# reglab/aquaculture

Hardware: AMD Instinct MI355X
Metric: 640px tiles/sec (whole node) YOLOv5m bf16 (higher is better)
Workload: dtype bf16

## Files before the change

aquaculture_amd/csrc/conv1x1_direct.hip:

```cpp
#include "conv_device.h"

using namespace aqdev;

namespace {

struct C1Params {
    const char* in;
    char* out;
    const char* w;
    const float* bias;
    const char* zero;
    int in_ld_b, out_ld_b;
    int npix, n_tiles, act;
    float out_inv_scale;
};

constexpr int kNW = 12;

template <int KS, int MBT, int MBW, int NBW> struct C1Geom {
    static constexpr int CIN = 32 * KS, COUT = 16 * MBT, CB = CIN / 8;
    static constexpr int MG = MBT / MBW;
    static constexpr int PG = kNW / MG;
    static constexpr int TP = PG * NBW * 16;
    static constexpr int SPP = CB + 2;
    static constexpr int PXB = SPP * 16;
    static constexpr int NQ = (TP * SPP + 63) / 64;
    static constexpr int XPB = NQ * 1024;
    static constexpr int LDS = 2 * XPB + COUT * 4;
    static constexpr int NST = NBW;
    static_assert(MBT % MBW == 0 && kNW % MG == 0 && LDS <= 160 * 1024, "shape");
};

__device__ __forceinline__ f32x4 c1_silu4(f32x4 v) {
    const f32x4 t = v * -1.44269504f;
    f32x4 d = {__builtin_amdgcn_exp2f(t[0]), __builtin_amdgcn_exp2f(t[1]), __builtin_amdgcn_exp2f(t[2]), __builtin_amdgcn_exp2f(t[3])};
    d = d + 1.0f;
    const f32x4 r = {__builtin_amdgcn_rcpf(d[0]), __builtin_amdgcn_rcpf(d[1]), __builtin_amdgcn_rcpf(d[2]), __builtin_amdgcn_rcpf(d[3])};
    return v * r;
}

template <int KS, int MBT, int MBW, int NBW, bool F8OUT = false>
__global__ __launch_bounds__(kNW * 64) void conv1x1_direct_kernel(const C1Params p) {
    using G = C1Geom<KS, MBT, MBW, NBW>;
    extern __shared__ __attribute__((aligned(16))) char smem[];
    float* s_b = (float*)(smem + 2 * G::XPB);

    const int tid = threadIdx.x, lane = tid & 63;
    const int wave = __builtin_amdgcn_readfirstlane(tid >> 6);
    static_assert(MBW == 2, "the paired-row layout below is written for two M blocks per wave");
    const int mb0 = (wave % G::MG) * MBW, pg = wave / G::MG;
    const int g = lane >> 4, l15 = lane & 15;
    const int cbase = mb0 * 16 + g * 8;

    bf16x8 wv[KS][MBW];
#pragma unroll
    for (int s = 0; s < KS; ++s)
#pragma unroll
        for (int m = 0; m < MBW; ++m) wv[s][m] = ((const bf16x8*)p.w)[((size_t)(mb0 + m) * KS + s) * 64 + lane];
    for (int i = tid; i < G::COUT; i += kNW * 64) s_b[i] = p.bias[i];

    auto issue_dma = [&](int tile, char* xb) {
        const long long n0 = (long long)tile * G::TP;
#pragma unroll 1
        for (int q = wave; q < G::NQ; q += kNW) {
            const int slot = q * 64 + lane;
            const int px = slot / G::SPP, part = slot - px * G::SPP;
            const bool valid = px < G::TP && part < G::CB && n0 + px < p.npix;
            const char* src = p.in + (n0 + px) * p.in_ld_b + part * 16;
            glds16(valid ? src : p.zero, xb + q * 1024);
        }
    };

    int tile = first_tile(gridDim.x, blockIdx.x);
    if (tile < p.n_tiles) issue_dma(tile, smem);
    int cur = 0;
    bool prev_full = false;
    for (; tile < p.n_tiles; tile += gridDim.x, cur ^= 1) {
        const long long n0 = (long long)tile * G::TP;
        const char* s_x = smem + cur * G::XPB;
        if (prev_full) wait_vmcnt<G::NST>(); else wait_vmcnt<0>();
        asm volatile("s_waitcnt lgkmcnt(0)" ::: "memory");
        __builtin_amdgcn_s_barrier();
        asm volatile("" ::: "memory");
        prev_full = n0 + G::TP <= p.npix;
        if (tile + (int)gridDim.x < p.n_tiles) issue_dma(tile + (int)gridDim.x, smem + (cur ^ 1) * G::XPB);

        f32x4 bv[MBW];
#pragma unroll
        for (int m = 0; m < MBW; ++m) bv[m] = *(const f32x4*)(s_b + cbase + m * 4);
        static_assert(G::NST == NBW * 1, "one 16-byte (8-byte with F8OUT) store per pixel block: the wait at the top of the tile loop counts these");
        AQ_STORE_LOOP_UNROLL
        for (int j = 0; j < NBW; ++j) {
            const int px = (pg * NBW + j) * 16 + l15;
            const char* base = s_x + px * G::PXB + g * 16;
            bf16x8 f[KS];
#pragma unroll
            for (int s = 0; s < KS; ++s) f[s] = *(const bf16x8*)(base + s * 64);
            f32x4 acc[MBW];
#pragma unroll
            for (int m = 0; m < MBW; ++m) acc[m] = f32x4{0.f, 0.f, 0.f, 0.f};
#pragma unroll
            for (int s = 0; s < KS; ++s)
#pragma unroll
                for (int m = 0; m < MBW; ++m) acc[m] = __builtin_amdgcn_mfma_f32_16x16x32_bf16(wv[s][m], f[s], acc[m], 0, 0, 0);
            f32x4 v0 = acc[0] + bv[0], v1 = acc[1] + bv[1];
            if (p.act) { v0 = c1_silu4(v0); v1 = c1_silu4(v1); }
            if constexpr (F8OUT) {
                f32x4 q0 = v0 * p.out_inv_scale, q1 = v1 * p.out_inv_scale;
#pragma unroll
                for (int e = 0; e < 4; ++e) {
                    q0[e] = __builtin_amdgcn_fmed3f(q0[e], -448.0f, 448.0f);
                    q1[e] = __builtin_amdgcn_fmed3f(q1[e], -448.0f, 448.0f);
                }
                int w0 = __builtin_amdgcn_cvt_pk_fp8_f32(q0[0], q0[1], 0, false);
                w0 = __builtin_amdgcn_cvt_pk_fp8_f32(q0[2], q0[3], w0, true);
                int w1 = __builtin_amdgcn_cvt_pk_fp8_f32(q1[0], q1[1], 0, false);
                w1 = __builtin_amdgcn_cvt_pk_fp8_f32(q1[2], q1[3], w1, true);
                if (n0 + px < p.npix) *(uint2*)(p.out + (n0 + px) * p.out_ld_b + cbase) = make_uint2((unsigned)w0, (unsigned)w1);
            } else if (n0 + px < p.npix)
                *(uint4*)(p.out + (n0 + px) * p.out_ld_b + cbase * 2) =
                    make_uint4(pack_bf16x2(v0[0], v0[1]), pack_bf16x2(v0[2], v0[3]), pack_bf16x2(v1[0], v1[1]), pack_bf16x2(v1[2], v1[3]));
        }
    }
}

template <int KS, int MBT, int MBW, int NBW, bool F8OUT = false>
int launch_c1(C1Params p, hipStream_t stream) {
    using G = C1Geom<KS, MBT, MBW, NBW>;
    auto fn = conv1x1_direct_kernel<KS, MBT, MBW, NBW, F8OUT>;
    int cus = 0;
    AQ_CHECK_HIP(aq_kernel_lds((const void*)fn, G::LDS));
    AQ_CHECK_HIP(aq_cus(&cus));
    p.n_tiles = (p.npix + G::TP - 1) / G::TP;
    long long grid = cus;
    if (grid > p.n_tiles) grid = p.n_tiles;
    hipLaunchKernelGGL(fn, dim3((unsigned)grid), dim3(kNW * 64), G::LDS, stream, p);
    AQ_CHECK_HIP(hipGetLastError());
    return AQ_OK;
}

}

extern "C" int aq_conv1x1_direct_supported(int cin, int cout) {
    return (cin == 96 && cout == 96) || (cin == 192 && cout == 192) || (cin == 384 && (cout == 192 || cout == 384));
}

extern "C" int aq_pack_conv1x1_direct(const float* w_host, int cin, int cout, void* packed_dev, size_t* bytes, void* stream) {
    AQ_REQUIRE(w_host && bytes && aq_conv1x1_direct_supported(cin, cout), "pack_conv1x1_direct: unsupported %d -> %d", cin, cout);
    const int ks = cin / 32, mbt = cout / 16;
    *bytes = (size_t)mbt * ks * 64 * 16;
    if (!packed_dev) return AQ_OK;
    bf16_t* host = (bf16_t*)calloc(1, *bytes);
    AQ_REQUIRE(host, "pack_conv1x1_direct: out of host memory");
    for (int mb = 0; mb < mbt; ++mb)
        for (int s = 0; s < ks; ++s)
            for (int lane = 0; lane < 64; ++lane) {
                const int r = lane & 15, g = lane >> 4;
                const int co = (mb >> 1) * 32 + 8 * (r >> 2) + 4 * (mb & 1) + (r & 3);
                bf16_t* dst = host + (((size_t)mb * ks + s) * 64 + lane) * 8;
                for (int e = 0; e < 8; ++e) dst[e] = aq_f2bf(w_host[(size_t)co * cin + 32 * s + 8 * g + e]);
            }
    hipError_t e = hipMemcpyAsync(packed_dev, host, *bytes, hipMemcpyHostToDevice, (hipStream_t)stream);
    if (e == hipSuccess) e = hipStreamSynchronize((hipStream_t)stream);
    free(host);
    AQ_CHECK_HIP(e);
    return AQ_OK;
}

extern "C" int aq_conv1x1_direct(const void* in_dev, int in_ld, int in_choff, void* out_dev, int out_ld, int out_choff, int cin, int cout,
                                 const void* packed_w_dev, const float* bias_dev, long long npix, int act, void* stream) {
    AQ_REQUIRE(in_dev && out_dev && packed_w_dev && bias_dev, "conv1x1_direct: null pointer");
    AQ_REQUIRE(aq_conv1x1_direct_supported(cin, cout), "conv1x1_direct: unsupported %d -> %d", cin, cout);
    AQ_REQUIRE(npix > 0 && npix < (1LL << 31), "conv1x1_direct: bad pixel count");
    AQ_REQUIRE(in_ld % 8 == 0 && out_ld % 8 == 0 && in_choff % 8 == 0 && out_choff % 8 == 0 && in_choff + cin <= in_ld && out_choff + cout <= out_ld,
               "conv1x1_direct: channel slices must be 8-aligned and inside their rows");
    C1Params p{};
    p.in = (const char*)in_dev + (size_t)in_choff * 2; p.in_ld_b = in_ld * 2;
    p.out = (char*)out_dev + (size_t)out_choff * 2; p.out_ld_b = out_ld * 2;
    p.w = (const char*)packed_w_dev; p.bias = bias_dev;
    p.npix = (int)npix; p.act = act;
    p.zero = aq_zero_page();
    AQ_REQUIRE(p.zero, "conv1x1_direct: zero page allocation failed");
    const hipStream_t st = (hipStream_t)stream;
    if (cin == 96) return launch_c1<3, 6, 2, 4>(p, st);
    if (cin == 192) return launch_c1<6, 12, 2, 4>(p, st);
    if (cout == 192) return launch_c1<12, 12, 2, 2>(p, st);
    return launch_c1<12, 24, 2, 4>(p, st);
}


extern "C" int aq_conv1x1_direct_f8out(const void* in_dev, int in_ld, int in_choff, void* out_dev, int out_pitch_bytes, int out_byte_off, int cin,
                                       int cout, const void* packed_w_dev, const float* bias_dev, long long npix, int act, float out_scale,
                                       void* stream) {
    AQ_REQUIRE(in_dev && out_dev && packed_w_dev && bias_dev, "conv1x1_direct_f8out: null pointer");
    AQ_REQUIRE((cin == 192 && cout == 192) || (cin == 384 && cout == 384), "conv1x1_direct_f8out: unsupported %d -> %d", cin, cout);
    AQ_REQUIRE(npix > 0 && npix < (1LL << 31) && out_scale > 0.0f, "conv1x1_direct_f8out: bad pixel count or scale");
    AQ_REQUIRE(in_ld % 8 == 0 && in_choff % 8 == 0 && in_choff + cin <= in_ld && out_pitch_bytes % 8 == 0 && out_byte_off % 8 == 0 &&
                   out_byte_off + cout <= out_pitch_bytes, "conv1x1_direct_f8out: slices must be 8-byte aligned and inside their rows");
    C1Params p{};
    p.in = (const char*)in_dev + (size_t)in_choff * 2; p.in_ld_b = in_ld * 2;
    p.out = (char*)out_dev + out_byte_off; p.out_ld_b = out_pitch_bytes;
    p.w = (const char*)packed_w_dev; p.bias = bias_dev;
    p.npix = (int)npix; p.act = act; p.out_inv_scale = 1.0f / out_scale;
    p.zero = aq_zero_page();
    AQ_REQUIRE(p.zero, "conv1x1_direct_f8out: zero page allocation failed");
    const hipStream_t st = (hipStream_t)stream;
    if (cin == 192) return launch_c1<6, 12, 2, 4, true>(p, st);
    return launch_c1<12, 24, 2, 4, true>(p, st);
}
```

aquaculture_amd/csrc/engine.cpp:

```cpp
#include "aq_common.h"
#include <unistd.h>
#include <string>

#include <cstdarg>
#include <cstdio>
#include <cstdlib>
#include <cstring>
#include <string>
#include <atomic>
#include <dlfcn.h>
#include <vector>

namespace {
thread_local char g_err[512] = "";
}

void aq_set_error(const char* fmt, ...) {
    va_list ap;
    va_start(ap, fmt);
    vsnprintf(g_err, sizeof(g_err), fmt, ap);
    va_end(ap);
}

extern "C" const char* aq_last_error(void) { return g_err; }
// ... 116 lines not shown
        }
    }
    *kgroups = kg; *kgroups_pad = kgp; *G = g; *cout_rows = rows;
}

struct TensorPlace { size_t offset = 0; size_t bytes = 0; int h = 0, w = 0, elem = 0; };

}

struct aq_engine {
    int device = 0;
    aq_model_desc desc{};
    std::vector<aq_tensor_desc> tensors;
    std::vector<aq_op_desc> ops;
    std::vector<PackedW> packed;
    std::vector<int> conv_cfg;
    int nms_agnostic = 0;
    unsigned long long nms_cls_lo = ~0ULL, nms_cls_hi = ~0ULL;
    struct Tuned { int B = 0, H = 0, W = 0; std::vector<int> cfg; };
    std::vector<Tuned> tuned;
    int tuned_cur = -1;
    bool tuning = false;
    void* zero_page = nullptr;
    int lay_B = 0, lay_H = 0, lay_W = 0;
    bool lay_aug = false;
    int run_H = 0, run_W = 0;
    std::vector<TensorPlace> place;
    size_t off_pred = 0, off_cand = 0, off_cand_rows = 0, off_cand_count = 0, off_cand_wide = 0, off_nms = 0, off_taps = 0, total_bytes = 0;
    int N = 0;
    aq_augment_pass aug[3] = {};
    std::vector<int> aug_family[3], aug_cfg[3];
    void* last_ws = nullptr;
    const uint8_t* last_tiles = nullptr;
    float* calib_amax = nullptr;
    std::vector<int> last_family, last_cfg;
    bool prof = false;
    int ring = 0;
    long long prof_calls = 0;
    std::vector<hipEvent_t> ev;
};

namespace {

void set_dims(aq_engine* e, int H, int W) {
    for (size_t t = 0; t < e->tensors.size(); ++t) {
        e->place[t].h = H / e->tensors[t].down;
        e->place[t].w = W / e->tensors[t].down;
    }
    e->run_H = H; e->run_W = W;
}

constexpr int kNmsRowLimit = 1 << 17;

int plan_unfit_op(const aq_engine* e, long long B, int H, int W, char* why, size_t why_len);

int layout(aq_engine* e, int B, int H, int W, bool aug = false) {
    AQ_REQUIRE(B > 0 && H >= 32 && W >= 32 && H % 32 == 0 && W % 32 == 0,
               "tile size must be a positive multiple of the max stride 32 (got B=%d H=%d W=%d)", B, H, W);
    if (e->lay_B == B && e->lay_H == H && e->lay_W == W && e->lay_aug == aug) {
        if (e->run_H != H || e->run_W != W) set_dims(e, H, W);
        return AQ_OK;
    }
    int n_aug = 0;
    aq_augment_pass passes[3] = {};
    if (aug) {
        const int rc = aq_augment_geometry(H, W, e->desc.na, passes, &n_aug);
// ... 253 lines not shown
            case AQ_CONV_CFG_PL3X3:
                form = B * (hs + 1) * (ws + 1) + ws + 2 < (1LL << 23) && npix * ld_d * 2 < (1LL << 31) && npix * ld_r * 2 < (1LL << 31);
                break;
            case AQ_CONV_CFG_PL3X3S2:
                form = B <= INT32_MAX && aq_conv3x3_pl_s2_supported(op.src.channels, op.dst.channels, (int)B, (int)hs, (int)ws) &&
                       npix * ld_d * 2 < (1LL << 31) && B * hs * ws * ld_s * 2 < (1LL << 31);
                break;
            default: form = false;
            }
            const bool forced = e->conv_cfg[oi] >= 0 && e->conv_cfg[oi] >= AQ_CONV_CFG_DIRECT1X1 && e->conv_cfg[oi] < AQ_CONV_CFG_ONE_TILE_PER_WG;
            if (!(form || (!forced && igemm))) return fail(oi, "conv: implicit-GEMM pixel count %lld >= 2^24 and no other form takes it", npix);
            break;
        }
        default:
            break;
        }
    }
    return -1;
}

bool c3tail_active(aq_engine* e, int oi, int last, int B) {
    if (!e->packed[oi].w_tail || oi + 1 >= last || e->calib_amax || e->tuning) return false;
    const int ci = oi + 1;
    const PackedW& pc = e->packed[ci];
    if (pc.direct_cfg != AQ_CONV_CFG_DIRECT1X1 || (pc.f8_consumer >= 0 && f8_pair_active(e, pc.f8_consumer, B))) return false;
    const aq_engine::Tuned* tt = tuned_for(e);
    const int cfg = e->conv_cfg[ci] >= 0 ? e->conv_cfg[ci] : tt ? tt->cfg[ci] : -1;
    if (cfg != AQ_CONV_CFG_DIRECT1X1) return false;
    const aq_op_desc& b = e->ops[oi];
    const aq_op_desc& c = e->ops[ci];
    const TensorPlace& pl = e->place[b.src.tensor];
    return aq_bottleneck_c3tail_supported(B, pl.h, pl.w, e->tensors[b.src.tensor].channels, e->tensors[c.src.tensor].channels,
                                          e->tensors[c.dst.tensor].channels) != 0;
}

struct AugRun {
    int pass;
    const aq_augment_pass* ps;
    int H0, W0;
    const aq_tap* ytab;
    const aq_tap* xtab;
};

int run_plan(aq_engine* e, const uint8_t* tiles, int B, int H, int W, void* ws, size_t ws_bytes,
             float* pred_out, aq_det* dets, int32_t* counts, float conf, float iou, int max_det, hipStream_t stream,
             int first = 0, int last = -1, const AugRun* ar = nullptr) {
    AQ_REQUIRE(e && tiles && ws, "infer: null pointer");
    const int n_ops = (int)e->ops.size();
    if (last < 0) last = n_ops;
    AQ_REQUIRE(0 <= first && first <= last && last <= n_ops, "run_ops: range [%d, %d) is not inside the plan's %d ops", first, last, n_ops);
    int rc = AQ_OK;
    if (!ar) {
        rc = layout(e, B, H, W);
        if (rc) return rc;
        if (ws_bytes < e->total_bytes) {
            aq_set_error("workspace too small: need %zu bytes, got %zu", e->total_bytes, ws_bytes);
            return AQ_ERR_WORKSPACE;
        }
    }
    const bool scaled = ar && ar->pass > 0;
    const int aug_base = ar ? ar->ps->out_first - ar->ps->keep_first : 0;
    const float aug_scale = ar ? ar->ps->scale : 1.0f, aug_flip_w = ar && ar->ps->flip ? (float)ar->W0 : 0.0f;
    e->last_ws = ws; e->last_tiles = tiles;
    const int prec = e->desc.precision;
    const bool whole = first == 0 && last == n_ops;
    hipEvent_t* ev = nullptr;
    if (whole && !ar && e->prof && e->ring > 0) ev = e->ev.data() + (size_t)(e->prof_calls % e->ring) * (n_ops + 1);
    float* pred = pred_out ? pred_out : (float*)((char*)ws + e->off_pred);
    int32_t* cand = (int32_t*)((char*)ws + e->off_cand);
    int32_t* cand_count = (int32_t*)((char*)ws + e->off_cand_count);
    float* cand_rows = (float*)((char*)ws + e->off_cand_rows);
    const char* use_sd = getenv("AQ_STEMDOWN");
    const bool stemdown = use_sd && *use_sd == '1' && prec == AQ_BF16 && n_ops > 2 && e->ops[0].kind == AQ_OP_STEM && e->ops[1].kind == AQ_OP_DOWNBLOCK &&
                          e->ops[0].dst.channels == 48 && e->ops[1].src.tensor == e->ops[0].dst.tensor && e->ops[1].src.ch_off == e->ops[0].dst.ch_off &&
                          aq_stemdown_supported(H, W) && ((uintptr_t)tiles & 3) == 0 && !scaled;
    const bool fuse_heads = dets != nullptr && heads_fused(e);
    bool heads_started = ar != nullptr;
    int heads_done = 0;
    for (int oi = 0; oi < first; ++oi)
        if (fuse_heads && e->ops[oi].kind == AQ_OP_CONV && e->ops[oi].level >= 0) {
            heads_started = true;
            ++heads_done;
        }
    int tail_conv = -1;
    for (int oi = first; oi < last; ++oi) {
        const aq_op_desc& op = e->ops[oi];
        if (ev) AQ_CHECK_HIP(hipEventRecord(ev[oi], stream));
        const bool mark = g_roctx.on();
        if (mark) {
            char name[96];
            snprintf(name, sizeof name, "aq op %02d kind %d: %d -> %d ch, k%d s%d%s", oi, op.kind, op.src.channels, op.dst.channels, op.k, op.stride,
                     op.level >= 0 ? " (detect head)" : "");
            g_roctx.push(name);
        }
        switch (op.kind) {
        case AQ_OP_PREPROCESS:
            if (scaled)
                rc = aq_preprocess_s2d_scaled(tiles, ar->H0, ar->W0, ar->ytab, ar->xtab, ar->ps->h, ar->ps->w, tptr(e, ws, tiles, op.dst.tensor), B, H, W,
                                              prec, stream);
            else
                rc = aq_preprocess_s2d(tiles, tptr(e, ws, tiles, op.dst.tensor), B, H, W, prec, stream);
            break;
        case AQ_OP_CONV:
            if (oi == tail_conv) {
                note_launch(e, oi, AQ_FAM_DIRECT1X1, AQ_CONV_CFG_DIRECT1X1);
                break;
            }
            if (ar && op.level >= 0 && !((ar->ps->level_mask >> op.level) & 1)) {
                note_launch(e, oi, AQ_FAM_NONE);
                break;
            }
            if (fuse_heads && op.level >= 0) {
                int32_t* wide = (int32_t*)((char*)ws + e->off_cand_wide);
                if (!heads_started) {
                    AQ_CHECK_HIP(hipMemsetAsync(wide, 0, sizeof(int32_t) * B * kCountStride, stream));
                    heads_started = true;
                }
                const TensorPlace& pl = e->place[op.src.tensor];
                int off = 0;
                for (int l = 0; l < op.level; ++l) off += e->desc.na * (H / (int)e->desc.stride[l]) * (W / (int)e->desc.stride[l]);
                float anchors[8 * 2];
                for (int a = 0; a < e->desc.na; ++a) {
                    anchors[2 * a] = e->desc.anchors_px[op.level][a][0];
                    anchors[2 * a + 1] = e->desc.anchors_px[op.level][a][1];
                }
                note_launch(e, oi, AQ_FAM_HEAD_DECODE);
                if (ar) {
                    rc = aq_head_decode_aug(tptr(e, ws, tiles, op.src.tensor), e->tensors[op.src.tensor].channels, op.src.ch_off, op.src.channels,
                                            e->packed[oi].w_head, B, pl.h, pl.w, aug_base + off, e->desc.stride[op.level], anchors, e->desc.nc, e->desc.na,
                                            conf, aug_scale, aug_flip_w, cand, cand_rows, wide, kCountStride, e->N, stream);
                    break;
                }
                rc = aq_head_decode(tptr(e, ws, tiles, op.src.tensor), e->tensors[op.src.tensor].channels, op.src.ch_off, op.src.channels,
                                    e->packed[oi].w_head, B, pl.h, pl.w, off, e->desc.stride[op.level], anchors, e->desc.nc, e->desc.na, conf,
                                    cand, cand_rows, wide, kCountStride, e->N, stream);
                if (!rc && ++heads_done == 3) rc = aq_head_counts_gather(wide, kCountStride, cand_count, B, stream);
// ... 27 lines not shown
                const aq_op_desc& c = e->ops[oi + 1];
                rc = aq_bottleneck_c3tail(tptr(e, ws, tiles, op.src.tensor), e->tensors[op.src.tensor].channels, op.src.ch_off,
                                          tptr(e, ws, tiles, c.src.tensor), e->tensors[c.src.tensor].channels, op.dst.channels,
                                          tptr(e, ws, tiles, c.dst.tensor), e->tensors[c.dst.tensor].channels, c.dst.ch_off,
                                          e->packed[oi].w_tail, e->packed[oi].b_tail, B, pl.h, pl.w, op.res.tensor >= 0, stream);
                tail_conv = oi + 1;
                break;
            }
            rc = aq_bottleneck(tptr(e, ws, tiles, op.src.tensor), e->tensors[op.src.tensor].channels, op.src.ch_off,
                               tptr(e, ws, tiles, op.dst.tensor), e->tensors[op.dst.tensor].channels, op.dst.ch_off,
                               op.src.channels, e->packed[oi].w, e->packed[oi].bias, B, pl.h, pl.w, op.res.tensor >= 0, stream);
            break;
        }
        case AQ_OP_DOWNBLOCK: {
            note_launch(e, oi, AQ_FAM_DOWNBLOCK);
            const TensorPlace& pl = e->place[op.src.tensor];
            if (stemdown && oi == 1) {
                rc = aq_stemdown(tiles, tptr(e, ws, tiles, op.dst.tensor), e->tensors[op.dst.tensor].channels, op.dst.ch_off,
                                 e->packed[0].w, e->packed[0].bias, e->packed[oi].w, e->packed[oi].bias, B, H, W, stream);
                break;
            }
            rc = aq_downblock(tptr(e, ws, tiles, op.src.tensor), e->tensors[op.src.tensor].channels, op.src.ch_off,
                              tptr(e, ws, tiles, op.dst.tensor), e->tensors[op.dst.tensor].channels, op.dst.ch_off,
                              e->packed[oi].w, e->packed[oi].bias, B, pl.h, pl.w, stream);
            break;
        }
        case AQ_OP_SPPF_POOL: {
            const TensorPlace& pl = e->place[op.src.tensor];
            rc = aq_sppf_pool(tptr(e, ws, tiles, op.src.tensor), e->tensors[op.src.tensor].channels, op.src.ch_off,
                              op.src.channels, B, pl.h, pl.w, prec, stream);
            break;
        }
        case AQ_OP_UPSAMPLE2X: {
            const TensorPlace& pl = e->place[op.src.tensor];
            rc = aq_upsample2x(tptr(e, ws, tiles, op.src.tensor), e->tensors[op.src.tensor].channels, op.src.ch_off,
                               tptr(e, ws, tiles, op.dst.tensor), e->tensors[op.dst.tensor].channels, op.dst.ch_off,
                               op.src.channels, B, pl.h, pl.w, prec, stream);
            break;
        }
        case AQ_OP_DECODE: {
            if (fuse_heads) break;
            const float* heads[3];
            for (int l = 0; l < 3; ++l) heads[l] = (const float*)tptr(e, ws, tiles, e->desc.head_tensor[l]);
            float anchors[3 * 8 * 2];
            for (int l = 0; l < 3; ++l)
                for (int a = 0; a < e->desc.na; ++a) {
                    anchors[(l * e->desc.na + a) * 2] = e->desc.anchors_px[l][a][0];
                    anchors[(l * e->desc.na + a) * 2 + 1] = e->desc.anchors_px[l][a][1];
                }
            const bool want_nms = dets != nullptr;
            if (ar) {
                rc = aq_detect_decode_aug(heads, e->tensors[e->desc.head_tensor[0]].channels, B, H, W, e->desc.nc, e->desc.na, anchors,
                                          e->desc.stride, ar->ps->level_mask, aug_base, e->N, aug_scale, aug_flip_w, want_nms ? nullptr : pred,
                                          conf, want_nms ? cand : nullptr, want_nms ? cand_rows : nullptr, want_nms ? cand_count : nullptr,
                                          e->N, stream);
                break;
            }
            rc = aq_detect_decode(heads, e->tensors[e->desc.head_tensor[0]].channels, B, H, W, e->desc.nc, e->desc.na,
                                  anchors, e->desc.stride, want_nms ? nullptr : pred, conf, want_nms ? cand : nullptr,
                                  want_nms ? cand_rows : nullptr, want_nms ? cand_count : nullptr, e->N, stream);
            break;
        }
        case AQ_OP_NMS:
            if (dets && !ar)
                rc = aq_nms_opts(cand_rows, e->N, B, e->N, e->desc.nc, conf, iou, max_det, cand, cand_count, e->N,
                                 (char*)ws + e->off_nms, dets, counts, e->nms_agnostic, e->nms_cls_lo, e->nms_cls_hi, stream);
// ... 350 lines not shown
                aq_pack_conv3x3_pl(op.weight, op.src.channels, op.dst.channels, pw.w_direct, &nb, nullptr) != AQ_OK) {
                aq_set_error("engine_create: planar 3x3 weight upload failed (op %zu)", oi);
                return fail(AQ_ERR_HIP);
            }
            pw.direct_cfg = AQ_CONV_CFG_PL3X3;
            const char* use_w8 = getenv("AQ_PL_W8");
            if (w8 && use_w8 && *use_w8 == '1') {
                if (aq_pack_conv3x3_pl_w8(op.weight, op.bias, op.src.channels, op.dst.channels, nullptr, &nb, nullptr, nullptr) == AQ_OK &&
                    hipMalloc(&pw.w_pl8, nb) == hipSuccess && hipMalloc((void**)&pw.sb_pl8, 2048 * sizeof(float)) == hipSuccess) {
                    if (aq_pack_conv3x3_pl_w8(op.weight, op.bias, op.src.channels, op.dst.channels, pw.w_pl8, &nb, pw.sb_pl8, nullptr) != AQ_OK) {
                        (void)hipFree(pw.w_pl8); (void)hipFree(pw.sb_pl8);
                        pw.w_pl8 = nullptr; pw.sb_pl8 = nullptr;
                    }
                }
            }
        }
        const char* no_hf = getenv("AQ_DISABLE_HEAD_FUSION");
        if (d->precision == AQ_BF16 && op.level >= 0 && op.k == 1 && op.stride == 1 && !op.act && op.res.tensor < 0 &&
            op.dst.channels >= d->na * (d->nc + 5) && op.dst.channels <= 32 && aq_head_decode_supported(op.src.channels, d->na, d->nc) && !(no_hf && *no_hf == '1')) {
            size_t nb = 0;
            if (aq_pack_head_weights(op.weight, op.bias, op.src.channels, op.dst.channels, nullptr, &nb, nullptr) != AQ_OK ||
                hipMalloc(&pw.w_head, nb) != hipSuccess ||
                aq_pack_head_weights(op.weight, op.bias, op.src.channels, op.dst.channels, pw.w_head, &nb, nullptr) != AQ_OK) {
                aq_set_error("engine_create: fused head weight upload failed (op %zu)", oi);
                return fail(AQ_ERR_HIP);
            }
        }
        if (d->precision == AQ_BF16 && op.kind == AQ_OP_CONV && op.k == 3 && op.stride == 1 && op.pad == 1 && e->packed[oi].direct_cfg == AQ_CONV_CFG_PL3X3 &&
            aq_conv3x3_pl_f8_supported(op.src.channels, op.dst.channels, 1, 8, 8)) {
            e->packed[oi].w_host.assign(op.weight, op.weight + (size_t)op.dst.channels * 9 * op.src.channels);
            e->packed[oi].b_host.assign(op.bias, op.bias + op.dst.channels);
        }
        op.weight = nullptr; op.bias = nullptr;
    }
    *out = e;
    return AQ_OK;
}

extern "C" void aq_engine_destroy(aq_engine* e) {
    if (!e) return;
    for (PackedW& pw : e->packed) {
        if (pw.w) (void)hipFree(pw.w);
        if (pw.w_direct) (void)hipFree(pw.w_direct);
        if (pw.w_head) (void)hipFree(pw.w_head);
        if (pw.w_pl8) (void)hipFree(pw.w_pl8);
        if (pw.w_f8) (void)hipFree(pw.w_f8);
        if (pw.sb_f8) (void)hipFree(pw.sb_f8);
        if (pw.sb_pl8) (void)hipFree(pw.sb_pl8);
        if (pw.w_tail) (void)hipFree(pw.w_tail);
        if (pw.b_tail) (void)hipFree(pw.b_tail);
        if (pw.bias) (void)hipFree(pw.bias);
    }
    if (e->zero_page) (void)hipFree(e->zero_page);
    for (hipEvent_t ev : e->ev) (void)hipEventDestroy(ev);
    delete e;
}

extern "C" int aq_engine_workspace_bytes(aq_engine* e, int max_batch, int H, int W, size_t* bytes) {
    AQ_REQUIRE(e && bytes, "workspace_bytes: null pointer");
    int rc = layout(e, max_batch, H, W);
    if (rc) return rc;
    *bytes = e->total_bytes;
    return AQ_OK;
}

extern "C" int aq_engine_infer(aq_engine* e, const uint8_t* tiles_dev, int B, int H, int W, void* ws, size_t ws_bytes,
// ... 318 lines not shown
```

aquaculture_amd/engine.py:

```python
from __future__ import annotations

import ctypes as C
import os
import re
from typing import Dict, List, Optional, Sequence, Tuple

import numpy as np
import torch

from . import spec as _spec
from .checkpoint import Checkpoint, pack_plan_weights

AQ_BF16, AQ_FP32, AQ_BF16_W8, AQ_F16X3 = 0, 1, 2, 3
PRECISIONS = {"bf16": AQ_BF16, "fp32": AQ_FP32, "fp8w": AQ_BF16, "f16x3": AQ_F16X3}
"""Compute precision of the single-op helpers.  fp8w = fp8 (OCP e4m3fn) weights with per-output-channel power-of-two scales, bf16
activations (quant.py): values bf16 holds exactly, so every bf16 kernel runs them as they are."""
ENGINE_PRECISIONS = {"bf16": AQ_BF16, "fp32": AQ_FP32, "fp8w": AQ_BF16_W8, "f16x3": AQ_F16X3, "fp8": AQ_BF16}
"""aq_model_desc.precision.  AQ_BF16_W8 computes as AQ_BF16; kernels with an fp8-weight stream (the planar 3x3) load the e4m3 codes."""
_DTYPE_CODE = {"act": 0, "f32": 1, "u8": 2}

LIB_PATH = os.path.join(os.path.dirname(os.path.abspath(__file__)), "csrc", "libaqengine.so")


class aq_tensor_desc(C.Structure):
    _fields_ = [("channels", C.c_int32), ("down", C.c_int32), ("dtype", C.c_int32)]


class aq_slice(C.Structure):
    _fields_ = [("tensor", C.c_int32), ("ch_off", C.c_int32), ("channels", C.c_int32)]


class aq_op_desc(C.Structure):
    _fields_ = [("kind", C.c_int32), ("src", aq_slice), ("dst", aq_slice), ("res", aq_slice),
                ("k", C.c_int32), ("stride", C.c_int32), ("pad", C.c_int32), ("act", C.c_int32),
                ("level", C.c_int32), ("weight", C.POINTER(C.c_float)), ("bias", C.POINTER(C.c_float)),
                ("flops_per_tile", C.c_double)]


class aq_model_desc(C.Structure):
    _fields_ = [("precision", C.c_int32), ("nc", C.c_int32), ("na", C.c_int32), ("nl", C.c_int32),
                ("anchors_px", C.c_float * 2 * 8 * 3), ("stride", C.c_float * 3),
                ("head_tensor", C.c_int32 * 3), ("input_tensor", C.c_int32),
                ("n_tensors", C.c_int32), ("n_ops", C.c_int32),
                ("tensors", C.POINTER(aq_tensor_desc)), ("ops", C.POINTER(aq_op_desc))]


class aq_det(C.Structure):
    _fields_ = [("x1", C.c_float), ("y1", C.c_float), ("x2", C.c_float), ("y2", C.c_float),
                ("conf", C.c_float), ("cls", C.c_float)]


EXPORTS = (
    "aq_last_error", "aq_version", "aq_engine_create", "aq_engine_destroy", "aq_engine_workspace_bytes",
    "aq_engine_infer", "aq_engine_run_ops", "aq_engine_candidates", "aq_engine_forward_raw", "aq_engine_tensor_ptr", "aq_engine_profile",
    "aq_engine_op_times", "aq_engine_num_ops", "aq_engine_set_conv_config", "aq_engine_autotune", "aq_engine_set_tuned_table",
    "aq_engine_get_conv_config", "aq_conv_num_configs", "aq_debug_conv_stamp", "aq_debug_mfma_peak",
    "aq_conv_config_tiles", "aq_pack_conv_weights", "aq_pack_conv_weights_x3", "aq_conv2d", "aq_pack_stem_weights", "aq_stem_conv", "aq_pack_bottleneck_weights", "aq_bottleneck", "aq_bottleneck_asm_form", "aq_bottleneck_c3tail_supported", "aq_pack_bottleneck_c3tail_weights", "aq_bottleneck_c3tail", "aq_pack_downblock_weights", "aq_downblock", "aq_stemdown_supported", "aq_stemdown", "aq_conv1x1_direct_supported", "aq_pack_conv1x1_direct", "aq_conv1x1_direct", "aq_conv1x1_asm_supported", "aq_pack_conv1x1_asm", "aq_conv1x1_asm", "aq_nms_opts", "aq_engine_set_nms_options",
    "aq_conv3x3s2_direct_supported", "aq_pack_conv3x3s2_direct", "aq_conv3x3s2_direct",
    "aq_conv3x3_pl_supported", "aq_conv3x3_pl_asm_family", "aq_pack_conv3x3_pl", "aq_conv3x3_pl", "aq_conv3x3_pl_s2_supported", "aq_pack_conv3x3_pl_s2", "aq_conv3x3_pl_s2", "aq_jpeg_scratch_bytes", "aq_jpeg_idct_rgb", "aq_f32_to_e4m3", "aq_conv1x1_direct_f8out", "aq_absmax_bf16", "aq_engine_calibrate_amax", "aq_engine_set_fp8_scales", "aq_engine_last_launch", "aq_conv3x3_pl_f8_supported", "aq_pack_conv3x3_pl_f8", "aq_conv3x3_pl_f8", "aq_conv3x3_pl_w8_supported", "aq_pack_conv3x3_pl_w8", "aq_conv3x3_pl_w8", "aq_head_decode_supported", "aq_pack_head_weights", "aq_head_decode", "aq_head_counts_gather", "aq_preprocess_s2d", "aq_sppf_pool",
    "aq_upsample2x", "aq_letterbox_u8", "aq_letterbox_tiles_u8", "aq_format_label_rows", "aq_detect_decode", "aq_nms_scratch_bytes", "aq_nms", "aq_jpeg_huffman_decode", "aq_write_label_files",
    "aq_crop_jpeg_coefs", "aq_crop_jpeg_bytes", "aq_write_crop_files",
    "aq_annotate_u8", "aq_image_jpeg_coefs", "aq_image_jpeg_bytes", "aq_write_image_files",
    "aq_blank_stats_scratch_bytes", "aq_blank_stats_u8",
    "aq_blank_geom_scratch_bytes", "aq_blank_components_u8", "aq_blank_ring_edges_u8",
    "aq_facility_scratch_bytes", "aq_facility_dbscan_f64",
    "aq_land_scratch_bytes", "aq_land_filter_f64",
    "aq_eval_scratch_bytes", "aq_eval_member_conf_f64", "aq_box_match_f64",
    "aq_augment_geometry", "aq_augment_taps", "aq_stem_conv_scaled", "aq_preprocess_s2d_scaled", "aq_head_decode_aug", "aq_detect_decode_aug",
    "aq_engine_workspace_bytes_augment", "aq_engine_infer_augment", "aq_engine_forward_raw_augment", "aq_engine_last_launch_augment",
)

_lib = None


def load_library(path: str = LIB_PATH) -> C.CDLL:
    global _lib
    if _lib is not None:
        return _lib
    if path == LIB_PATH and os.environ.get("AQ_ENGINE_LIB"):
        path = os.environ["AQ_ENGINE_LIB"]
    if not os.path.exists(path):
        raise RuntimeError(f"{path} not found: build it with `python -m aquaculture_amd.build` "
                           "(there is no CPU/PyTorch fallback for the detect path)")
    lib = C.CDLL(path)
    vp, i32, f32, sz = C.c_void_p, C.c_int, C.c_float, C.c_size_t
    lib.aq_last_error.restype = C.c_char_p
    lib.aq_engine_create.argtypes = [C.POINTER(aq_model_desc), i32, C.POINTER(vp)]
    lib.aq_engine_destroy.argtypes = [vp]
    lib.aq_engine_destroy.restype = None
    lib.aq_engine_workspace_bytes.argtypes = [vp, i32, i32, i32, C.POINTER(sz)]
# ... 35 lines not shown
    lib.aq_facility_dbscan_f64.argtypes = [vp, vp, vp, vp, C.c_longlong, C.c_double, i32, vp, sz, vp, vp, vp]
    lib.aq_land_scratch_bytes.argtypes = [C.c_longlong]
    lib.aq_land_scratch_bytes.restype = sz
    lib.aq_land_filter_f64.argtypes = [vp, C.c_longlong, vp, C.c_longlong, vp, i32, C.c_double, C.c_double, vp, C.c_longlong, vp, sz, vp, vp]
    lib.aq_eval_scratch_bytes.argtypes = [C.c_longlong, i32]
    lib.aq_eval_scratch_bytes.restype = sz
    lib.aq_eval_member_conf_f64.argtypes = [vp, vp, vp, vp, vp, C.c_longlong, C.c_double, i32, vp, sz, vp, vp]
    lib.aq_box_match_f64.argtypes = [vp, vp, C.c_longlong, vp, C.c_longlong, vp, i32, vp, i32, vp, vp, vp]
    lib.aq_engine_set_tuned_table.argtypes = [vp, i32, i32, i32, C.POINTER(i32), i32]
    lib.aq_engine_calibrate_amax.argtypes = [vp, vp, i32, i32, i32, vp, sz, C.POINTER(f32), i32, vp]
    lib.aq_engine_set_fp8_scales.argtypes = [vp, C.POINTER(f32), i32]
    lib.aq_conv1x1_direct_f8out.argtypes = [vp, i32, i32, vp, i32, i32, i32, i32, vp, vp, C.c_longlong, i32, f32, vp]
    lib.aq_absmax_bf16.argtypes = [vp, i32, i32, i32, C.c_longlong, vp, vp]
    lib.aq_debug_conv_stamp.argtypes = [vp, sz]
    lib.aq_debug_mfma_peak.argtypes = [i32, i32, vp, vp]
    lib.aq_conv_config_tiles.argtypes = [i32, C.POINTER(i32), C.POINTER(i32)]
    lib.aq_pack_conv_weights.argtypes = [C.POINTER(f32), i32, i32, i32, i32, vp, C.POINTER(sz), vp]
    lib.aq_pack_conv_weights_x3.argtypes = [C.POINTER(f32), C.POINTER(f32), i32, i32, i32, vp, C.POINTER(sz), vp, C.POINTER(sz), vp]
    lib.aq_conv2d.argtypes = [vp, i32, i32, i32, vp, i32, i32, i32, vp, i32, i32, vp, vp,
                              i32, i32, i32, i32, i32, i32, i32, i32, i32, vp, vp]
    lib.aq_pack_stem_weights.argtypes = [C.POINTER(f32), i32, i32, vp, C.POINTER(sz), vp]
    lib.aq_stem_conv.argtypes = [vp, vp, i32, i32, i32, vp, vp, i32, i32, i32, i32, i32, vp]
    lib.aq_pack_bottleneck_weights.argtypes = [C.POINTER(f32), C.POINTER(f32), i32, vp, C.POINTER(sz), vp]
    lib.aq_bottleneck.argtypes = [vp, i32, i32, vp, i32, i32, i32, vp, vp, i32, i32, i32, i32, vp]
    lib.aq_bottleneck_asm_form.argtypes = [i32] * 6
    lib.aq_bottleneck_c3tail_supported.argtypes = [i32, i32, i32, i32, i32, i32]
    lib.aq_pack_bottleneck_c3tail_weights.argtypes = [C.POINTER(f32), C.POINTER(f32), C.POINTER(f32), vp, C.POINTER(sz), vp]
    lib.aq_bottleneck_c3tail.argtypes = [vp, i32, i32, vp, i32, i32, vp, i32, i32, vp, vp, i32, i32, i32, i32, vp]
    lib.aq_pack_downblock_weights.argtypes = [C.POINTER(f32), C.POINTER(f32), vp, C.POINTER(sz), vp]
    lib.aq_downblock.argtypes = [vp, i32, i32, vp, i32, i32, vp, vp, i32, i32, i32, vp]
    lib.aq_conv1x1_direct_supported.argtypes = [i32, i32]
    lib.aq_pack_conv1x1_direct.argtypes = [C.POINTER(f32), i32, i32, vp, C.POINTER(sz), vp]
    lib.aq_conv1x1_direct.argtypes = [vp, i32, i32, vp, i32, i32, i32, i32, vp, vp, C.c_longlong, i32, vp]
    lib.aq_nms_opts.argtypes = [vp, i32, i32, i32, i32, f32, f32, i32, vp, vp, i32, vp, vp, vp, i32, C.c_ulonglong, C.c_ulonglong, vp]
    lib.aq_engine_set_nms_options.argtypes = [vp, i32, C.c_ulonglong, C.c_ulonglong]
    lib.aq_conv1x1_asm_supported.argtypes = [i32, i32]
    lib.aq_pack_conv1x1_asm.argtypes = [C.POINTER(f32), i32, i32, vp, C.POINTER(sz), vp]
    lib.aq_conv1x1_asm.argtypes = [vp, i32, i32, vp, i32, i32, i32, i32, vp, vp, C.c_longlong, i32, vp]
    lib.aq_conv3x3s2_direct_supported.argtypes = [i32, i32]
    lib.aq_pack_conv3x3s2_direct.argtypes = [C.POINTER(f32), i32, i32, vp, C.POINTER(sz), vp]
    lib.aq_conv3x3s2_direct.argtypes = [vp, i32, i32, vp, i32, i32, i32, i32, vp, vp, i32, i32, i32, i32, vp]
    lib.aq_conv3x3_pl_supported.argtypes = [i32, i32]
    lib.aq_conv3x3_pl_asm_family.argtypes = [i32]
    lib.aq_pack_conv3x3_pl.argtypes = [C.POINTER(f32), i32, i32, vp, C.POINTER(sz), vp]
    lib.aq_conv3x3_pl.argtypes = [vp, C.c_longlong, C.c_longlong, i32, vp, i32, i32, i32, vp, i32, i32, vp, vp, i32, i32, i32, i32, vp]
    lib.aq_conv3x3_pl_w8.argtypes = lib.aq_conv3x3_pl.argtypes
    lib.aq_pack_conv3x3_pl_w8.argtypes = [C.POINTER(C.c_float), C.POINTER(C.c_float), i32, i32, vp, C.POINTER(C.c_size_t), vp, vp]
    lib.aq_conv3x3_pl_w8_supported.argtypes = [i32] * 5
    lib.aq_jpeg_scratch_bytes.argtypes = [i32, i32, i32]
    lib.aq_jpeg_scratch_bytes.restype = sz
    lib.aq_jpeg_idct_rgb.argtypes = [vp, vp, vp, i32, i32, i32, vp, vp, vp]
    lib.aq_f32_to_e4m3.argtypes = [f32]
    lib.aq_f32_to_e4m3.restype = C.c_ubyte
    lib.aq_conv3x3_pl_f8_supported.argtypes = [i32] * 5
    lib.aq_pack_conv3x3_pl_f8.argtypes = [C.POINTER(f32), C.POINTER(f32), i32, i32, f32, vp, C.POINTER(sz), vp, vp]
    lib.aq_conv3x3_pl_f8.argtypes = [vp, i32, i32, i32, vp, i32, i32, i32, vp, i32, i32, vp, vp, i32, i32, i32, i32, vp]
    lib.aq_conv3x3_pl_s2_supported.argtypes = [i32] * 5
    lib.aq_pack_conv3x3_pl_s2.argtypes = [C.POINTER(f32), i32, i32, vp, C.POINTER(sz), vp]
    lib.aq_conv3x3_pl_s2.argtypes = [vp, i32, i32, i32, vp, i32, i32, i32, vp, vp, i32, i32, i32, i32, vp]
    lib.aq_preprocess_s2d.argtypes = [vp, vp, i32, i32, i32, i32, vp]
    lib.aq_sppf_pool.argtypes = [vp, i32, i32, i32, i32, i32, i32, i32, vp]
    lib.aq_upsample2x.argtypes = [vp, i32, i32, vp, i32, i32, i32, i32, i32, i32, i32, vp]
    lib.aq_letterbox_u8.argtypes = [vp, i32, i32, i32, vp, i32, i32, i32, i32, i32, i32, vp, vp, vp]
    lib.aq_letterbox_tiles_u8.argtypes = [vp, C.c_longlong, C.c_longlong, vp, vp, i32, i32, i32, vp, i32, i32, i32, i32, i32, i32, vp, vp, vp]
    lib.aq_format_label_rows.argtypes = [C.POINTER(f32), i32, i32, C.c_char_p, sz]
    lib.aq_format_label_rows.restype = C.c_long
# ... 1582 lines not shown
```

include/aq_engine.h:

```cpp
#ifndef AQ_ENGINE_H
#define AQ_ENGINE_H

#include <stddef.h>
#include <stdint.h>

#ifdef __cplusplus
extern "C" {
#endif

typedef enum aq_status {
    AQ_OK = 0,
    AQ_ERR_INVALID = -1,
    AQ_ERR_HIP = -2,
    AQ_ERR_NOMEM = -3,
    AQ_ERR_WORKSPACE = -4
} aq_status;

typedef enum aq_precision {
    AQ_BF16 = 0,
    AQ_FP32 = 1,
    AQ_BF16_W8 = 2,
    AQ_F16X3 = 3
} aq_precision;

// ... 98 lines not shown
              const void* res_dev, int res_ld, int res_choff,
              const void* packed_w_dev, const float* bias_dev,
              int B, int H, int W, int k, int stride, int pad, int act,
              int precision, int out_f32, const void* zero_page_dev, void* stream);
int aq_pack_stem_weights(const float* w_krsc_host, int cout, int precision, void* packed_dev, size_t* bytes, void* stream);
int aq_stem_conv(const uint8_t* tiles_dev, void* out_dev, int out_ld, int out_choff, int cout, const void* packed_w_dev,
                 const float* bias_dev, int B, int H, int W, int act, int precision, void* stream);

int aq_pack_bottleneck_weights(const float* w1_host, const float* w2_host, int C, void* packed_dev, size_t* bytes, void* stream);
int aq_bottleneck(const void* in_dev, int in_ld, int in_choff, void* out_dev, int out_ld, int out_choff, int C,
                  const void* packed_w_dev, const float* bias_dev, int B, int H, int W, int shortcut, void* stream);
int aq_bottleneck_asm_form(int C, int B, int H, int W, int in_ld, int out_ld);

int aq_bottleneck_c3tail_supported(int B, int H, int W, int in_ld, int cat_ld, int out_ld);
int aq_pack_bottleneck_c3tail_weights(const float* w1_host, const float* w2_host, const float* w3_host, void* packed_dev, size_t* bytes,
                                      void* stream);
int aq_bottleneck_c3tail(const void* in_dev, int in_ld, int in_choff, const void* cat_dev, int cat_ld, int cat_choff, void* out_dev,
                         int out_ld, int out_choff, const void* packed_w_dev, const float* bias_dev, int B, int H, int W, int shortcut,
                         void* stream);

int aq_pack_downblock_weights(const float* wa_host, const float* wb_host, void* packed_dev, size_t* bytes, void* stream);
int aq_downblock(const void* in_dev, int in_ld, int in_choff, void* out_dev, int out_ld, int out_choff,
                 const void* packed_w_dev, const float* bias_dev, int B, int H, int W, void* stream);
int aq_stemdown_supported(int Hi, int Wi);
int aq_stemdown(const uint8_t* tiles_dev, void* out_dev, int out_ld, int out_choff, const void* stem_w_dev, const float* stem_bias_dev,
                const void* packed_w_dev, const float* bias_dev, int B, int Hi, int Wi, void* stream);

#define AQ_CONV_CFG_DIRECT1X1 1000
#define AQ_CONV_CFG_ONE_TILE_PER_WG 4096
int aq_conv1x1_direct_supported(int cin, int cout);
int aq_pack_conv1x1_direct(const float* w_host, int cin, int cout, void* packed_dev, size_t* bytes, void* stream);
int aq_conv1x1_direct(const void* in_dev, int in_ld, int in_choff, void* out_dev, int out_ld, int out_choff, int cin, int cout,
                      const void* packed_w_dev, const float* bias_dev, long long npix, int act, void* stream);

#define AQ_CONV_CFG_ASM1X1 1004
int aq_conv1x1_asm_supported(int cin, int cout);
int aq_pack_conv1x1_asm(const float* w_host, int cin, int cout, void* packed_dev, size_t* bytes, void* stream);
int aq_conv1x1_asm(const void* in_dev, int in_ld, int in_choff, void* out_dev, int out_ld, int out_choff, int cin, int cout,
                   const void* packed_w_dev, const float* bias_dev, long long npix, int act, void* stream);

#define AQ_CONV_CFG_DIRECT3X3S2 1001
int aq_conv3x3s2_direct_supported(int cin, int cout);
int aq_pack_conv3x3s2_direct(const float* w_host, int cin, int cout, void* packed_dev, size_t* bytes, void* stream);
int aq_conv3x3s2_direct(const void* in_dev, int in_ld, int in_choff, void* out_dev, int out_ld, int out_choff, int cin, int cout,
                        const void* packed_w_dev, const float* bias_dev, int B, int H, int W, int act, void* stream);
#define AQ_CONV_CFG_PL3X3 1002
int aq_conv3x3_pl_supported(int cin, int cout);
int aq_conv3x3_pl_asm_family(int nb);
int aq_pack_conv3x3_pl(const float* w_krsc_host, int cin, int cout, void* packed_dev, size_t* bytes, void* stream);
int aq_conv3x3_pl(const void* in_dev, long long in_pixel_stride_b, long long in_group_stride_b, int cin,
                  void* out_dev, int out_ld, int out_choff, int cout, const void* res_dev, int res_ld, int res_choff,
                  const void* packed_w_dev, const float* bias_dev, int B, int H, int W, int act, void* stream);
#define AQ_CONV_CFG_PL3X3S2 1003
int aq_conv3x3_pl_s2_supported(int cin, int cout, int B, int H, int W);
int aq_pack_conv3x3_pl_s2(const float* w_krsc_host, int cin, int cout, void* packed_dev, size_t* bytes, void* stream);
int aq_conv3x3_pl_s2(const void* in_dev, int in_ld, int in_choff, int cin, void* out_dev, int out_ld, int out_choff, int cout,
                     const void* packed_w_dev, const float* bias_dev, int B, int H, int W, int act, void* stream);
int aq_conv1x1_direct_f8out(const void* in_dev, int in_ld, int in_choff, void* out_dev, int out_pitch_bytes, int out_byte_off, int cin, int cout,
                            const void* packed_w_dev, const float* bias_dev, long long npix, int act, float out_scale, void* stream);
int aq_absmax_bf16(const void* t_dev, int ld, int choff, int c, long long npix, float* out_dev, void* stream);
unsigned char aq_f32_to_e4m3(float v);
int aq_conv3x3_pl_f8_supported(int cin, int cout, int B, int H, int W);
int aq_pack_conv3x3_pl_f8(const float* w_krsc_host, const float* bias_host, int cin, int cout, float act_scale, void* packed_dev,
                          size_t* bytes, float* scale_bias_dev, void* stream);
int aq_conv3x3_pl_f8(const void* in_dev, int in_ld, int in_choff, int cin, void* out_dev, int out_ld, int out_choff, int cout,
                     const void* res_dev, int res_ld, int res_choff, const void* packed_w_dev, const float* scale_bias_dev,
// ... 135 lines not shown
```

Measured before the change: 17070.

## Fold nearest 2x upsample into following direct 1x1 conv input loads

Adds an UP variant of the direct 1x1 conv kernel that reads the upsampled channel slice straight from the low-resolution tensor via a computed source-pixel index, so the separate upsample2x kernel launch and its full-resolution write/read are skipped. The engine detects upsample->conv pairs (384-channel concat input, tensor not read elsewhere) at build time and enables the fold by default for bf16 unless AQ_UPFOLD=0. The cost is an integer divide per DMA slot for index computation and less coalesced gathers from the low-res tensor.

```diff
diff --git a/aquaculture_amd/csrc/conv1x1_direct.hip b/aquaculture_amd/csrc/conv1x1_direct.hip
--- a/aquaculture_amd/csrc/conv1x1_direct.hip
+++ b/aquaculture_amd/csrc/conv1x1_direct.hip
@@ -1,4 +1,6 @@
 #include "conv_device.h"
+#include "up2x_index.h"
+#include <type_traits>
 
 using namespace aqdev;
 
@@ -14,6 +16,13 @@
     int npix, n_tiles, act;
     float out_inv_scale;
 };
+
+struct C1UpParams : C1Params {
+    const char* up_in;
+    int up_ld_b, up_cb;
+    int H, W;
+};
+template <bool UP> using C1P = std::conditional_t<UP, C1UpParams, C1Params>;
 
 constexpr int kNW = 12;
 
@@ -39,8 +48,8 @@
     return v * r;
 }
 
-template <int KS, int MBT, int MBW, int NBW, bool F8OUT = false>
-__global__ __launch_bounds__(kNW * 64) void conv1x1_direct_kernel(const C1Params p) {
+template <int KS, int MBT, int MBW, int NBW, bool F8OUT = false, bool UP = false>
+__global__ __launch_bounds__(kNW * 64) void conv1x1_direct_kernel(const C1P<UP> p) {
     using G = C1Geom<KS, MBT, MBW, NBW>;
     extern __shared__ __attribute__((aligned(16))) char smem[];
     float* s_b = (float*)(smem + 2 * G::XPB);
@@ -67,6 +76,10 @@
             const int px = slot / G::SPP, part = slot - px * G::SPP;
             const bool valid = px < G::TP && part < G::CB && n0 + px < p.npix;
             const char* src = p.in + (n0 + px) * p.in_ld_b + part * 16;
+            if constexpr (UP) {
+                if (part < p.up_cb)
+                    src = p.up_in + aq_up2x_source_pixel((unsigned)(n0 + px), (unsigned)p.H, (unsigned)p.W) * p.up_ld_b + part * 16;
+            }
             glds16(valid ? src : p.zero, xb + q * 1024);
         }
     };
@@ -124,10 +137,10 @@
     }
 }
 
-template <int KS, int MBT, int MBW, int NBW, bool F8OUT = false>
-int launch_c1(C1Params p, hipStream_t stream) {
+template <int KS, int MBT, int MBW, int NBW, bool F8OUT = false, bool UP = false>
+int launch_c1(C1P<UP> p, hipStream_t stream) {
     using G = C1Geom<KS, MBT, MBW, NBW>;
-    auto fn = conv1x1_direct_kernel<KS, MBT, MBW, NBW, F8OUT>;
+    auto fn = conv1x1_direct_kernel<KS, MBT, MBW, NBW, F8OUT, UP>;
     int cus = 0;
     AQ_CHECK_HIP(aq_kernel_lds((const void*)fn, G::LDS));
     AQ_CHECK_HIP(aq_cus(&cus));
@@ -188,6 +201,32 @@
     return launch_c1<12, 24, 2, 4>(p, st);
 }
 
+extern "C" int aq_conv1x1_direct_up2x(const void* up_dev, int up_ld, int up_choff, int up_c, const void* in_dev, int in_ld, int in_choff,
+                                      void* out_dev, int out_ld, int out_choff, int cin, int cout, const void* packed_w_dev,
+                                      const float* bias_dev, int B, int H, int W, int act, void* stream) {
+    AQ_REQUIRE(up_dev && in_dev && out_dev && packed_w_dev && bias_dev, "conv1x1_direct_up2x: null pointer");
+    AQ_REQUIRE(cin == 384 && (cout == 192 || cout == 384), "conv1x1_direct_up2x: unsupported %d -> %d", cin, cout);
+    AQ_REQUIRE(B > 0 && H > 0 && W > 0 && H % 2 == 0 && W % 2 == 0, "conv1x1_direct_up2x: H and W must be positive and even (got %d x %d x %d)", B, H, W);
+    const long long npix = (long long)B * H * W;
+    AQ_REQUIRE(npix < (1LL << 31), "conv1x1_direct_up2x: bad pixel count");
+    AQ_REQUIRE(up_c % 8 == 0 && up_c > 0 && up_c < cin, "conv1x1_direct_up2x: %d of %d channels from the low-resolution tensor", up_c, cin);
+    AQ_REQUIRE(in_ld % 8 == 0 && out_ld % 8 == 0 && in_choff % 8 == 0 && out_choff % 8 == 0 && in_choff >= 0 && out_choff >= 0 &&
+                   in_choff + cin <= in_ld && out_choff + cout <= out_ld && up_ld % 8 == 0 && up_choff % 8 == 0 && up_choff >= 0 &&
+                   up_choff + up_c <= up_ld,
+               "conv1x1_direct_up2x: channel slices must be 8-aligned and inside their rows");
+    C1UpParams p{};
+    p.in = (const char*)in_dev + (size_t)in_choff * 2; p.in_ld_b = in_ld * 2;
+    p.out = (char*)out_dev + (size_t)out_choff * 2; p.out_ld_b = out_ld * 2;
+    p.up_in = (const char*)up_dev + (size_t)up_choff * 2; p.up_ld_b = up_ld * 2; p.up_cb = up_c / 8;
+    p.H = H; p.W = W;
+    p.w = (const char*)packed_w_dev; p.bias = bias_dev;
+    p.npix = (int)npix; p.act = act;
+    p.zero = aq_zero_page();
+    AQ_REQUIRE(p.zero, "conv1x1_direct_up2x: zero page allocation failed");
+    const hipStream_t st = (hipStream_t)stream;
+    if (cout == 192) return launch_c1<12, 12, 2, 2, false, true>(p, st);
+    return launch_c1<12, 24, 2, 4, false, true>(p, st);
+}
 
 extern "C" int aq_conv1x1_direct_f8out(const void* in_dev, int in_ld, int in_choff, void* out_dev, int out_pitch_bytes, int out_byte_off, int cin,
                                        int cout, const void* packed_w_dev, const float* bias_dev, long long npix, int act, float out_scale,
diff --git a/aquaculture_amd/csrc/engine.cpp b/aquaculture_amd/csrc/engine.cpp
--- a/aquaculture_amd/csrc/engine.cpp
+++ b/aquaculture_amd/csrc/engine.cpp
@@ -172,6 +172,7 @@
     std::vector<int> aug_family[3], aug_cfg[3];
     void* last_ws = nullptr;
     const uint8_t* last_tiles = nullptr;
+    std::vector<char> upfold;
     float* calib_amax = nullptr;
     std::vector<int> last_family, last_cfg;
     bool prof = false;
@@ -491,6 +492,19 @@
     const TensorPlace& pl = e->place[b.src.tensor];
     return aq_bottleneck_c3tail_supported(B, pl.h, pl.w, e->tensors[b.src.tensor].channels, e->tensors[c.src.tensor].channels,
                                           e->tensors[c.dst.tensor].channels) != 0;
+}
+
+bool upfold_active(aq_engine* e, int oi, int last, int B) {
+    if (e->upfold.empty() || !e->upfold[oi] || oi + 1 >= last || e->calib_amax || e->tuning) return false;
+    const int ci = oi + 1;
+    const PackedW& pc = e->packed[ci];
+    if (pc.direct_cfg != AQ_CONV_CFG_DIRECT1X1 || (pc.f8_consumer >= 0 && f8_pair_active(e, pc.f8_consumer, B))) return false;
+    const aq_engine::Tuned* tt = tuned_for(e);
+    const int cfg = e->conv_cfg[ci] >= 0 ? e->conv_cfg[ci] : tt ? tt->cfg[ci] : -1;
+    if (cfg != AQ_CONV_CFG_DIRECT1X1) return false;
+    const TensorPlace& lo = e->place[e->ops[oi].src.tensor];
+    const TensorPlace& hi = e->place[e->ops[ci].src.tensor];
+    return hi.h == 2 * lo.h && hi.w == 2 * lo.w && (long long)B * hi.h * hi.w < (1LL << 31);
 }
 
 struct AugRun {
@@ -542,6 +556,7 @@
             ++heads_done;
         }
     int tail_conv = -1;
+    int up_conv = -1;
     for (int oi = first; oi < last; ++oi) {
         const aq_op_desc& op = e->ops[oi];
         if (ev) AQ_CHECK_HIP(hipEventRecord(ev[oi], stream));
@@ -561,6 +576,16 @@
                 rc = aq_preprocess_s2d(tiles, tptr(e, ws, tiles, op.dst.tensor), B, H, W, prec, stream);
             break;
         case AQ_OP_CONV:
+            if (oi == up_conv) {
+                const aq_op_desc& u = e->ops[oi - 1];
+                const TensorPlace& pd = e->place[op.dst.tensor];
+                note_launch(e, oi, AQ_FAM_DIRECT1X1, AQ_CONV_CFG_DIRECT1X1);
+                rc = aq_conv1x1_direct_up2x(tptr(e, ws, tiles, u.src.tensor), e->tensors[u.src.tensor].channels, u.src.ch_off, u.src.channels,
+                                            tptr(e, ws, tiles, op.src.tensor), e->tensors[op.src.tensor].channels, op.src.ch_off,
+                                            tptr(e, ws, tiles, op.dst.tensor), e->tensors[op.dst.tensor].channels, op.dst.ch_off,
+                                            op.src.channels, op.dst.channels, e->packed[oi].w_direct, e->packed[oi].bias, B, pd.h, pd.w, op.act, stream);
+                break;
+            }
             if (oi == tail_conv) {
                 note_launch(e, oi, AQ_FAM_DIRECT1X1, AQ_CONV_CFG_DIRECT1X1);
                 break;
@@ -654,6 +679,10 @@
             break;
         }
         case AQ_OP_UPSAMPLE2X: {
+            if (upfold_active(e, oi, last, B)) {
+                up_conv = oi + 1;
+                break;
+            }
             const TensorPlace& pl = e->place[op.src.tensor];
             rc = aq_upsample2x(tptr(e, ws, tiles, op.src.tensor), e->tensors[op.src.tensor].channels, op.src.ch_off,
                                tptr(e, ws, tiles, op.dst.tensor), e->tensors[op.dst.tensor].channels, op.dst.ch_off,
@@ -1070,6 +1099,26 @@
             e->packed[oi].b_host.assign(op.bias, op.bias + op.dst.channels);
         }
         op.weight = nullptr; op.bias = nullptr;
+    }
+    const char* use_fold = getenv("AQ_UPFOLD");
+    e->upfold.assign(e->ops.size(), 0);
+    for (size_t oi = 0; d->precision == AQ_BF16 && !(use_fold && *use_fold == '0') && oi + 1 < e->ops.size(); ++oi) {
+        const aq_op_desc& u = e->ops[oi];
+        const aq_op_desc& c = e->ops[oi + 1];
+        if (u.kind != AQ_OP_UPSAMPLE2X || c.kind != AQ_OP_CONV || e->packed[oi + 1].direct_cfg != AQ_CONV_CFG_DIRECT1X1) continue;
+        if (u.dst.ch_off != 0 || u.dst.channels != u.src.channels || u.src.tensor == u.dst.tensor || u.src.channels % 8 || u.src.ch_off % 8 ||
+            e->tensors[u.src.tensor].channels % 8 || e->tensors[u.src.tensor].dtype != AQ_T_ACT || e->tensors[u.dst.tensor].dtype != AQ_T_ACT)
+            continue;
+        if (c.src.tensor != u.dst.tensor || c.src.ch_off != 0 || c.src.channels != e->tensors[c.src.tensor].channels || c.src.channels != 384 ||
+            u.dst.channels >= c.src.channels || c.dst.tensor == u.src.tensor || c.dst.tensor == c.src.tensor || c.level >= 0)
+            continue;
+        bool read_elsewhere = false;
+        for (size_t oj = 0; oj < e->ops.size(); ++oj) {
+            if (oj == oi + 1 || e->ops[oj].kind == AQ_OP_DECODE || e->ops[oj].kind == AQ_OP_NMS) continue;
+            for (const aq_slice* s : {&e->ops[oj].src, &e->ops[oj].res})
+                if (s->tensor == u.dst.tensor && s->ch_off < u.dst.ch_off + u.dst.channels && u.dst.ch_off < s->ch_off + s->channels) read_elsewhere = true;
+        }
+        if (!read_elsewhere) e->upfold[oi] = 1;
     }
     *out = e;
     return AQ_OK;
diff --git a/aquaculture_amd/csrc/up2x_index.h b/aquaculture_amd/csrc/up2x_index.h
--- /dev/null
+++ b/aquaculture_amd/csrc/up2x_index.h
@@ -0,0 +1,14 @@
+#pragma once
+
+#if defined(__HIPCC__)
+#define AQ_UP2X_HD __host__ __device__ __forceinline__
+#else
+#define AQ_UP2X_HD inline
+#endif
+
+AQ_UP2X_HD long long aq_up2x_source_pixel(unsigned n, unsigned H, unsigned W) {
+    const unsigned hw = H * W;
+    const unsigned b = n / hw, r = n - b * hw;
+    const unsigned y = r / W, x = r - y * W;
+    return (long long)b * (H >> 1) * (W >> 1) + (y >> 1) * (W >> 1) + (x >> 1);
+}
diff --git a/aquaculture_amd/engine.py b/aquaculture_amd/engine.py
--- a/aquaculture_amd/engine.py
+++ b/aquaculture_amd/engine.py
@@ -55,7 +55,7 @@
     "aq_engine_infer", "aq_engine_run_ops", "aq_engine_candidates", "aq_engine_forward_raw", "aq_engine_tensor_ptr", "aq_engine_profile",
     "aq_engine_op_times", "aq_engine_num_ops", "aq_engine_set_conv_config", "aq_engine_autotune", "aq_engine_set_tuned_table",
     "aq_engine_get_conv_config", "aq_conv_num_configs", "aq_debug_conv_stamp", "aq_debug_mfma_peak",
-    "aq_conv_config_tiles", "aq_pack_conv_weights", "aq_pack_conv_weights_x3", "aq_conv2d", "aq_pack_stem_weights", "aq_stem_conv", "aq_pack_bottleneck_weights", "aq_bottleneck", "aq_bottleneck_asm_form", "aq_bottleneck_c3tail_supported", "aq_pack_bottleneck_c3tail_weights", "aq_bottleneck_c3tail", "aq_pack_downblock_weights", "aq_downblock", "aq_stemdown_supported", "aq_stemdown", "aq_conv1x1_direct_supported", "aq_pack_conv1x1_direct", "aq_conv1x1_direct", "aq_conv1x1_asm_supported", "aq_pack_conv1x1_asm", "aq_conv1x1_asm", "aq_nms_opts", "aq_engine_set_nms_options",
+    "aq_conv_config_tiles", "aq_pack_conv_weights", "aq_pack_conv_weights_x3", "aq_conv2d", "aq_pack_stem_weights", "aq_stem_conv", "aq_pack_bottleneck_weights", "aq_bottleneck", "aq_bottleneck_asm_form", "aq_bottleneck_c3tail_supported", "aq_pack_bottleneck_c3tail_weights", "aq_bottleneck_c3tail", "aq_pack_downblock_weights", "aq_downblock", "aq_stemdown_supported", "aq_stemdown", "aq_conv1x1_direct_supported", "aq_pack_conv1x1_direct", "aq_conv1x1_direct", "aq_conv1x1_direct_up2x", "aq_conv1x1_asm_supported", "aq_pack_conv1x1_asm", "aq_conv1x1_asm", "aq_nms_opts", "aq_engine_set_nms_options",
     "aq_conv3x3s2_direct_supported", "aq_pack_conv3x3s2_direct", "aq_conv3x3s2_direct",
     "aq_conv3x3_pl_supported", "aq_conv3x3_pl_asm_family", "aq_pack_conv3x3_pl", "aq_conv3x3_pl", "aq_conv3x3_pl_s2_supported", "aq_pack_conv3x3_pl_s2", "aq_conv3x3_pl_s2", "aq_jpeg_scratch_bytes", "aq_jpeg_idct_rgb", "aq_f32_to_e4m3", "aq_conv1x1_direct_f8out", "aq_absmax_bf16", "aq_engine_calibrate_amax", "aq_engine_set_fp8_scales", "aq_engine_last_launch", "aq_conv3x3_pl_f8_supported", "aq_pack_conv3x3_pl_f8", "aq_conv3x3_pl_f8", "aq_conv3x3_pl_w8_supported", "aq_pack_conv3x3_pl_w8", "aq_conv3x3_pl_w8", "aq_head_decode_supported", "aq_pack_head_weights", "aq_head_decode", "aq_head_counts_gather", "aq_preprocess_s2d", "aq_sppf_pool",
     "aq_upsample2x", "aq_letterbox_u8", "aq_letterbox_tiles_u8", "aq_format_label_rows", "aq_detect_decode", "aq_nms_scratch_bytes", "aq_nms", "aq_jpeg_huffman_decode", "aq_write_label_files",
@@ -157,6 +157,7 @@
     lib.aq_conv1x1_direct_supported.argtypes = [i32, i32]
     lib.aq_pack_conv1x1_direct.argtypes = [C.POINTER(f32), i32, i32, vp, C.POINTER(sz), vp]
     lib.aq_conv1x1_direct.argtypes = [vp, i32, i32, vp, i32, i32, i32, i32, vp, vp, C.c_longlong, i32, vp]
+    lib.aq_conv1x1_direct_up2x.argtypes = [vp, i32, i32, i32, vp, i32, i32, vp, i32, i32, i32, i32, vp, vp, i32, i32, i32, i32, vp]
     lib.aq_nms_opts.argtypes = [vp, i32, i32, i32, i32, f32, f32, i32, vp, vp, i32, vp, vp, vp, i32, C.c_ulonglong, C.c_ulonglong, vp]
     lib.aq_engine_set_nms_options.argtypes = [vp, i32, C.c_ulonglong, C.c_ulonglong]
     lib.aq_conv1x1_asm_supported.argtypes = [i32, i32]
diff --git a/include/aq_engine.h b/include/aq_engine.h
--- a/include/aq_engine.h
+++ b/include/aq_engine.h
@@ -154,6 +154,9 @@
 int aq_pack_conv1x1_direct(const float* w_host, int cin, int cout, void* packed_dev, size_t* bytes, void* stream);
 int aq_conv1x1_direct(const void* in_dev, int in_ld, int in_choff, void* out_dev, int out_ld, int out_choff, int cin, int cout,
                       const void* packed_w_dev, const float* bias_dev, long long npix, int act, void* stream);
+int aq_conv1x1_direct_up2x(const void* up_dev, int up_ld, int up_choff, int up_c, const void* in_dev, int in_ld, int in_choff,
+                           void* out_dev, int out_ld, int out_choff, int cin, int cout, const void* packed_w_dev, const float* bias_dev,
+                           int B, int H, int W, int act, void* stream);
 
 #define AQ_CONV_CFG_ASM1X1 1004
 int aq_conv1x1_asm_supported(int cin, int cout);
```

Result: no change. 16970 (-0.6%).
